# RomanArzumanyan/VALI

Hardware: AMD Instinct MI355X
Metric: nv12_to_rgb_2160p_frames_per_s (higher is better)
Workload: dtype u8; 1 GPU; BatchedFramePipeline / PySurfaceConverter.RunBatch NV12->RGB 3840x2160, BT.709 limited range, 512 frames/GPU per step (BASELINE configs[4] geometry); frames_per_gpu=512, global_batch=512, bytes_per_frame=37324800, parallelism=frame-sharded x1, RCCL broadcast of coefficients

## Files before the change

### vali_amd/csrc/common.hpp

```cpp
#pragma once
#include <hip/hip_runtime.h>
#include <stdint.h>
#include <stdio.h>
#include <string>

#include "../../include/vali_hip.h"

namespace vali {

std::string& last_error();

int fail(int code, const char* fmt, ...) __attribute__((format(printf, 2, 3)));

class DeviceScope {
public:
  explicit DeviceScope(int device);
  ~DeviceScope();
  bool ok() const { return m_ok; }

private:
  int m_prev = -1;
  bool m_switched = false;
  bool m_ok = true;
};

int stream_device(hipStream_t stream);

unsigned residency_lds_bytes(int block_threads, int waves_per_cu, unsigned min_bytes);

inline int streaming_waves_per_cu(int groups, int block, int full_lane_waves) {
  const int lanes = ((groups + block - 1) / block) * block;
  const int util_pct = groups * 100 / lanes;
  return util_pct >= 90 ? full_lane_waves : util_pct >= 70 ? full_lane_waves * 3 / 2 : full_lane_waves * 7 / 4;
}

int tuning(int key);

class TraceRange {
public:
  explicit TraceRange(const char* name);
  ~TraceRange();

private:
  bool m_pushed = false;
};

inline hipStream_t as_stream(vali_stream_t s) { return (hipStream_t)s; }

inline bool aligned16(const void* p) { return (((uintptr_t)p) & 15u) == 0; }

inline bool planes_fit_32bit(const vali_surface& s) {
  for (int c = 0; c < 3; ++c)
    if (s.plane[c] && (s.pitch[c] < 0 || (uint64_t)s.pitch[c] * (uint64_t)s.height * 3u >= (1ull << 32)))
      return false;
  return true;
}

inline bool subsampled_sizes_ok(int format, int width, int height) {
  switch (format) {
  case VALI_FMT_NV12: case VALI_FMT_P10: case VALI_FMT_P12: case VALI_FMT_YUV420: case VALI_FMT_YUV420_10BIT:
    return ((width | height) & 1) == 0;
  case VALI_FMT_YUV422:
    return (width & 1) == 0;
  default:
    return true;
  }
}

}

#define VALI_ENTRY_NAMED(stream, name)                                                       \
  ::vali::TraceRange _trace(name);                                                            \
  const int _dev = ::vali::stream_device(stream);                                             \
  if (_dev < 0)                                                                               \
    return ::vali::fail(VALI_ERR_NO_DEVICE, "%s: no usable HIP device", name);                \
  ::vali::DeviceScope scope(_dev);                                                            \
  if (!scope.ok())                                                                            \
    return ::vali::fail(VALI_ERR_NO_DEVICE, "%s: cannot select device %d", name, _dev)
#define VALI_ENTRY(stream) VALI_ENTRY_NAMED(stream, __func__)

#define VALI_HIP_CHECK(expr)                                                   \
  do {                                                                         \
    hipError_t _e = (expr);                                                    \
    if (_e != hipSuccess)                                                      \
      return ::vali::fail(VALI_ERR_RUNTIME, "%s failed: %s (%s:%d)", #expr,    \
                          hipGetErrorString(_e), __FILE__, __LINE__);          \
  } while (0)

#define VALI_REQUIRE(cond, msg)                                                \
  do {                                                                         \
    if (!(cond))                                                               \
      return ::vali::fail(VALI_ERR_INVALID_ARG, "%s: %s", __func__, msg);      \
  } while (0)

#define VALI_LAUNCH_CHECK()                                                    \
  do {                                                                         \
    hipError_t _e = hipGetLastError();                                         \
    if (_e != hipSuccess)                                                      \
      return ::vali::fail(VALI_ERR_RUNTIME, "%s: kernel launch failed: %s",    \
                          __func__, hipGetErrorString(_e));                    \
  } while (0)
```

### vali_amd/csrc/cvt_nv12_rgb.hip

```cpp
#include "common.hpp"
#include "dev_util.hpp"

namespace vali {

enum : int { LAYOUT_RGB = 0, LAYOUT_BGR = 1, LAYOUT_PLANAR = 2 };

struct Nv12RgbArgs {
  const vali_surface* d_src;
  const vali_surface* d_dst;
  vali_surface src;
  vali_surface dst;
  vali_csc csc;
  TileMap map;
  int rp;
};

template <int LAYOUT>
__device__ __forceinline__ void emit4(u32 y4, const ChromaTerm& c01, const ChromaTerm& c23,
                                      const vali_csc& k, u32* o3, u32& pr, u32& pg,
                                      u32& pb) {
  const float y0 = luma_term(ubyte_f32<0>(y4), k), y1 = luma_term(ubyte_f32<1>(y4), k),
              y2 = luma_term(ubyte_f32<2>(y4), k), y3 = luma_term(ubyte_f32<3>(y4), k);
  const float r0 = y0 + c01.rv, g0 = y0 + c01.guv, b0 = y0 + c01.bu;
  const float r1 = y1 + c01.rv, g1 = y1 + c01.guv, b1 = y1 + c01.bu;
  const float r2 = y2 + c23.rv, g2 = y2 + c23.guv, b2 = y2 + c23.bu;
  const float r3 = y3 + c23.rv, g3 = y3 + c23.guv, b3 = y3 + c23.bu;
  if constexpr (LAYOUT == LAYOUT_PLANAR) {
    u32 r = 0, g = 0, b = 0;
    r = pack_u8<0>(r0, r); r = pack_u8<1>(r1, r); r = pack_u8<2>(r2, r); r = pack_u8<3>(r3, r);
    g = pack_u8<0>(g0, g); g = pack_u8<1>(g1, g); g = pack_u8<2>(g2, g); g = pack_u8<3>(g3, g);
    b = pack_u8<0>(b0, b); b = pack_u8<1>(b1, b); b = pack_u8<2>(b2, b); b = pack_u8<3>(b3, b);
    pr = r; pg = g; pb = b;
  } else {
    const float f0 = LAYOUT == LAYOUT_RGB ? r0 : b0, l0 = LAYOUT == LAYOUT_RGB ? b0 : r0;
    const float f1 = LAYOUT == LAYOUT_RGB ? r1 : b1, l1 = LAYOUT == LAYOUT_RGB ? b1 : r1;
    const float f2 = LAYOUT == LAYOUT_RGB ? r2 : b2, l2 = LAYOUT == LAYOUT_RGB ? b2 : r2;
    const float f3 = LAYOUT == LAYOUT_RGB ? r3 : b3, l3 = LAYOUT == LAYOUT_RGB ? b3 : r3;
    u32 d0 = 0, d1 = 0, d2 = 0;
    d0 = pack_u8<0>(f0, d0); d0 = pack_u8<1>(g0, d0); d0 = pack_u8<2>(l0, d0); d0 = pack_u8<3>(f1, d0);
    d1 = pack_u8<0>(g1, d1); d1 = pack_u8<1>(l1, d1); d1 = pack_u8<2>(f2, d1); d1 = pack_u8<3>(g2, d1);
    d2 = pack_u8<0>(l2, d2); d2 = pack_u8<1>(f3, d2); d2 = pack_u8<2>(g3, d2); d2 = pack_u8<3>(l3, d2);
    o3[0] = d0; o3[1] = d1; o3[2] = d2;
  }
}

template <int LAYOUT>
__device__ __forceinline__ void convert_group(const uint4& ya, const uint4& yb, const uint4& uv, const vali_csc& k,
                                              u32 (&o0)[12], u32 (&o1)[12]) {
  const u32 yw0[4] = {ya.x, ya.y, ya.z, ya.w};
  const u32 yw1[4] = {yb.x, yb.y, yb.z, yb.w};
  const u32 uvw[4] = {uv.x, uv.y, uv.z, uv.w};
#pragma unroll
  for (int j = 0; j < 4; ++j) {
    const ChromaTerm c01 = chroma_term(ubyte_f32<0>(uvw[j]), ubyte_f32<1>(uvw[j]), k);
    const ChromaTerm c23 = chroma_term(ubyte_f32<2>(uvw[j]), ubyte_f32<3>(uvw[j]), k);
    if constexpr (LAYOUT == LAYOUT_PLANAR) {
      emit4<LAYOUT>(yw0[j], c01, c23, k, nullptr, o0[j], o0[4 + j], o0[8 + j]);
      emit4<LAYOUT>(yw1[j], c01, c23, k, nullptr, o1[j], o1[4 + j], o1[8 + j]);
    } else {
      u32 dummy;
      emit4<LAYOUT>(yw0[j], c01, c23, k, &o0[3 * j], dummy, dummy, dummy);
      emit4<LAYOUT>(yw1[j], c01, c23, k, &o1[3 * j], dummy, dummy, dummy);
    }
  }
}

template <int LAYOUT>
__global__ void __launch_bounds__(kBlock) k_nv12_rgb8(const Nv12RgbArgs a) {
  extern __shared__ uint4 dyn_lds[];
  PackedStrip* const strips = reinterpret_cast<PackedStrip*>(dyn_lds);

  u32 tile_x, tile_y, frame;
  if (!tile_of_block(a.map, tile_x, tile_y, frame))
    return;

  const uint8_t* py;
  const uint8_t* puv;
  uint8_t* pd0;
  uint8_t* pd1;
  uint8_t* pd2;
  int sp_y, sp_uv, dp, W, H;
  if (a.d_src) {
    const vali_surface* s = a.d_src + frame;
    const vali_surface* d = a.d_dst + frame;
    py = (const uint8_t*)s->plane[0]; puv = (const uint8_t*)s->plane[1];
    sp_y = s->pitch[0]; sp_uv = s->pitch[1]; W = s->width; H = s->height;
    pd0 = (uint8_t*)d->plane[0]; pd1 = (uint8_t*)d->plane[1]; pd2 = (uint8_t*)d->plane[2];
    dp = d->pitch[0];
  } else {
    py = (const uint8_t*)a.src.plane[0]; puv = (const uint8_t*)a.src.plane[1];
    sp_y = a.src.pitch[0]; sp_uv = a.src.pitch[1]; W = a.src.width; H = a.src.height;
    pd0 = (uint8_t*)a.dst.plane[0]; pd1 = (uint8_t*)a.dst.plane[1]; pd2 = (uint8_t*)a.dst.plane[2];
    dp = a.dst.pitch[0];
  }
  const vali_csc k = a.csc;

  const int lane = threadIdx.x & (kWave - 1);
  const int wave_all = threadIdx.x / kWave;
  const int wpr = (int)(blockDim.x / kWave) / a.rp;
  const int wave = wave_all;
  const int wave_g0 = (tile_x * wpr + wave_all % wpr) * kWave;
  const int groups = (W + kLanePx - 1) / kLanePx;
  if (wave_g0 >= groups)
    return;
  const int g = wave_g0 + lane;
  const int x0 = g * kLanePx;
  const int crow = tile_y * a.rp + wave_all / wpr;
  if (crow * 2 >= H)
    return;
  const int row0 = crow * 2;

  uintptr_t align_bits = (uintptr_t)py | (uintptr_t)puv | (uintptr_t)sp_y |
                         (uintptr_t)sp_uv | (uintptr_t)pd0 | (uintptr_t)dp;
  if constexpr (LAYOUT == LAYOUT_PLANAR)
    align_bits |= (uintptr_t)pd1 | (uintptr_t)pd2;
  const bool fast = ((W & (kLanePx - 1)) == 0) && ((align_bits & 15u) == 0);

  if (fast) {
    const bool lane_valid = g < groups;
    u32 o0[12], o1[12];
    if (lane_valid) {
      const uint4 ya = load16(py + (size_t)row0 * sp_y + x0);
      const uint4 yb = load16(py + (size_t)(row0 + 1) * sp_y + x0);
      const uint4 uv = load16(puv + (size_t)crow * sp_uv + x0);
      convert_group<LAYOUT>(ya, yb, uv, k, o0, o1);
    }
    if constexpr (LAYOUT == LAYOUT_PLANAR) {
      if (lane_valid) {
        uint8_t* const planes[3] = {pd0, pd1, pd2};
#pragma unroll
        for (int c = 0; c < 3; ++c) {
          uint8_t* p = planes[c] + (size_t)row0 * dp + x0;
          store16_nt(p, make_uint4(o0[4 * c], o0[4 * c + 1], o0[4 * c + 2], o0[4 * c + 3]));
          store16_nt(p + dp, make_uint4(o1[4 * c], o1[4 * c + 1], o1[4 * c + 2], o1[4 * c + 3]));
        }
      }
    } else {
      PackedStrip& strip = strips[wave];
      const int valid_lanes = min(kWave, groups - wave_g0);
      const int valid_bytes = valid_lanes * 48;
      uint8_t* rb = pd0 + (size_t)row0 * dp + (size_t)wave_g0 * 48;
      strip_store_row(strip, lane, o0, lane_valid, rb, valid_bytes);
      strip_store_row(strip, lane, o1, lane_valid, rb + dp, valid_bytes);
    }
    return;
  }

  {
    const bool lane_valid = g < groups;
    const bool cut = lane_valid && x0 + kLanePx > W;
    const int xs = cut ? max(W - kLanePx, 0) : x0;
    const int n_px = min(kLanePx, W);
    u32 o0[12], o1[12];
    if (lane_valid) {
      const uint4 ya = load16_n(py + (size_t)row0 * sp_y + xs, n_px);
      const uint4 yb = load16_n(py + (size_t)(row0 + 1) * sp_y + xs, n_px);
      const uint4 uv = load16_n(puv + (size_t)crow * sp_uv + xs, n_px);
      convert_group<LAYOUT>(ya, yb, uv, k, o0, o1);
    }
    if constexpr (LAYOUT == LAYOUT_PLANAR) {
      if (lane_valid) {
        uint8_t* const planes[3] = {pd0, pd1, pd2};
#pragma unroll
        for (int c = 0; c < 3; ++c) {
          uint8_t* p = planes[c] + (size_t)row0 * dp + xs;
          store16_n(p, make_uint4(o0[4 * c], o0[4 * c + 1], o0[4 * c + 2], o0[4 * c + 3]), n_px);
          store16_n(p + dp, make_uint4(o1[4 * c], o1[4 * c + 1], o1[4 * c + 2], o1[4 * c + 3]), n_px);
        }
      }
    } else {
      PackedStrip& strip = strips[wave];
      const int full_lanes = min(kWave, W / kLanePx - wave_g0);
      uint8_t* rb = pd0 + (size_t)row0 * dp + (size_t)wave_g0 * 48;
      strip_store_row_u(strip, lane, o0, lane_valid && !cut, rb, full_lanes * 48);
      strip_store_row_u(strip, lane, o1, lane_valid && !cut, rb + dp, full_lanes * 48);
      if (cut) {
        packed_group_store(pd0 + (size_t)row0 * dp + (size_t)xs * 3, n_px, o0);
        packed_group_store(pd0 + (size_t)(row0 + 1) * dp + (size_t)xs * 3, n_px, o1);
      }
    }
  }
}

static int launch_nv12_rgb(Nv12RgbArgs& a, int width, int height, int n, int dst_format,
                           hipStream_t stream) {
  const int groups = (width + kLanePx - 1) / kLanePx;
  int block = ((groups + kWave - 1) / kWave) * kWave;
  if (block > kBlock)
    block = kBlock;
  const int rp_env = tuning(VALI_TUNE_NV12_ROWPAIRS);
  const int row_block = block;
  a.rp = rp_env > 0 ? rp_env : kBlock / row_block;
  if (a.rp < 1 || row_block * a.rp > kBlock)
    a.rp = 1;
  a.map = make_tile_map((groups + row_block - 1) / row_block, ((height + 1) / 2 + a.rp - 1) / a.rp, (u32)n);
  block = row_block * a.rp;
  const dim3 grid = tile_grid(a.map);
  const int waves_override = tuning(VALI_TUNE_WAVES_PER_CU);
  const int waves_per_cu = waves_override > 0 ? waves_override : streaming_waves_per_cu(groups, row_block, 16);
  const unsigned lds =
      residency_lds_bytes(block, waves_per_cu, (unsigned)sizeof(PackedStrip) * (unsigned)((block + kWave - 1) / kWave));
  switch (dst_format) {
  case VALI_FMT_RGB:
    hipLaunchKernelGGL((k_nv12_rgb8<LAYOUT_RGB>), grid, dim3(block), lds, stream, a);
    break;
  case VALI_FMT_BGR:
    hipLaunchKernelGGL((k_nv12_rgb8<LAYOUT_BGR>), grid, dim3(block), lds, stream, a);
    break;
  case VALI_FMT_RGB_PLANAR:
    hipLaunchKernelGGL((k_nv12_rgb8<LAYOUT_PLANAR>), grid, dim3(block), lds, stream, a);
    break;
  default:
    return fail(VALI_ERR_UNSUPPORTED, "nv12_to_rgb: unsupported dst format %d", dst_format);
  }
  VALI_LAUNCH_CHECK();
  return VALI_OK;
}

}

using namespace vali;

extern "C" {

int vali_nv12_to_rgb(const vali_surface* src, const vali_surface* dst, const vali_csc* csc,
                     vali_stream_t stream) {
  VALI_REQUIRE(src && dst && csc, "null argument");
  VALI_REQUIRE(src->format == VALI_FMT_NV12, "src must be NV12");
  VALI_REQUIRE(src->width > 0 && src->height > 0, "empty src");
  VALI_REQUIRE(src->width == dst->width && src->height == dst->height, "src/dst size mismatch");
  VALI_REQUIRE(((src->width | src->height) & 1) == 0, "4:2:0 surfaces need even width and height");
  VALI_REQUIRE(src->plane[0] && src->plane[1] && dst->plane[0], "null plane");
  if (dst->format == VALI_FMT_RGB_PLANAR)
    VALI_REQUIRE(dst->plane[1] && dst->plane[2], "null planar plane");
  Nv12RgbArgs a = {};
  a.src = *src;
  a.dst = *dst;
  a.csc = *csc;
  hipStream_t s = as_stream(stream);
  VALI_ENTRY(s);
  return launch_nv12_rgb(a, src->width, src->height, 1, dst->format, s);
}

int vali_nv12_to_rgb_batch(const vali_surface* d_src, const vali_surface* d_dst, int n, int width,
                           int height, int dst_format, const vali_csc* csc,
                           vali_stream_t stream) {
  VALI_REQUIRE(d_src && d_dst && csc, "null argument");
  VALI_REQUIRE(width > 0 && height > 0, "empty geometry");
  VALI_REQUIRE(((width | height) & 1) == 0, "4:2:0 surfaces need even width and height");
  VALI_REQUIRE(n >= 0 && n <= 65535, "batch size out of range (0..65535)");
  if (n == 0)
    return VALI_OK;
  Nv12RgbArgs a = {};
  a.d_src = d_src;
  a.d_dst = d_dst;
  a.csc = *csc;
  hipStream_t s = as_stream(stream);
  VALI_ENTRY(s);
  return launch_nv12_rgb(a, width, height, n, dst_format, s);
}


__global__ void k_debug_quantize(const float* in, uint8_t* out, int n) {
  const int i = blockIdx.x * blockDim.x + threadIdx.x;
  if (i < n)
    out[i] = (uint8_t)quantize_u8(in[i]);
}

__global__ void k_debug_quantize_portable(const float* in, uint8_t* out, int n) {
  const int i = blockIdx.x * blockDim.x + threadIdx.x;
  if (i < n)
    out[i] = (uint8_t)quantize_u8_portable(in[i]);
}

int vali_debug_quantize_u8(const float* d_in, uint8_t* d_out, int n, vali_stream_t stream) {
  VALI_REQUIRE(d_in && d_out && n >= 0, "bad argument");
  if (!n)
    return VALI_OK;
  hipStream_t s = as_stream(stream);
  VALI_ENTRY(s);
  hipLaunchKernelGGL(k_debug_quantize, dim3((n + 255) / 256), dim3(256), 0, s, d_in, d_out, n);
  VALI_LAUNCH_CHECK();
  return VALI_OK;
}

int vali_debug_quantize_u8_portable(const float* d_in, uint8_t* d_out, int n,
                                    vali_stream_t stream) {
  VALI_REQUIRE(d_in && d_out && n >= 0, "bad argument");
  if (!n)
    return VALI_OK;
  hipStream_t s = as_stream(stream);
  VALI_ENTRY(s);
  hipLaunchKernelGGL(k_debug_quantize_portable, dim3((n + 255) / 256), dim3(256), 0, s, d_in,
                     d_out, n);
  VALI_LAUNCH_CHECK();
  return VALI_OK;
}

}
```

### vali_amd/csrc/dev_util.hpp

```cpp
#pragma once
#include <hip/hip_runtime.h>
#include <stdint.h>

#include <type_traits>

#include "../../include/vali_hip.h"

namespace vali {

typedef uint32_t u32;

constexpr int kLanePx = 16;
constexpr int kWave = 64;
constexpr int kBlock = 256;
constexpr int kWavesPerBlock = kBlock / kWave;

template <int I> __device__ __forceinline__ float ubyte_f32(u32 w) {
  return (float)((w >> (8 * I)) & 0xffu);
}

template <int I> __device__ __forceinline__ u32 ubyte(u32 w) {
  return (w >> (8 * I)) & 0xffu;
}

__device__ __forceinline__ u32 quantize_u8_portable(float v) {
  float r = __builtin_rintf(v);
  r = __builtin_fminf(__builtin_fmaxf(r, 0.0f), 255.0f);
  return (u32)r;
}

template <int SEL> __device__ __forceinline__ u32 pack_u8(float v, u32 old) {
  return __builtin_amdgcn_cvt_pk_u8_f32(v, SEL, old);
}

__device__ __forceinline__ u32 quantize_u8(float v) { return __builtin_amdgcn_cvt_pk_u8_f32(v, 0, 0u); }

struct ChromaTerm {
  float rv, guv, bu;
};

__device__ __forceinline__ ChromaTerm chroma_term(float u, float v, const vali_csc& k) {
  const float uc = u - 128.0f, vc = v - 128.0f;
  ChromaTerm t;
  t.rv = k.crv * vc;
  t.guv = __builtin_fmaf(k.cgu, uc, k.cgv * vc);
  t.bu = k.cbu * uc;
  return t;
}

__device__ __forceinline__ float luma_term(float y, const vali_csc& k) {
  return k.cy * (y - k.y0);
}

struct Lerp {
  int i0, i1;
  float a;
};

__device__ __forceinline__ Lerp make_lerp(int x, float scale, int size) {
  const float f = (float)x * scale;
  const float fl = __builtin_floorf(f);
  Lerp l;
  l.a = f - fl;
  const int i = (int)fl;
  l.i0 = min(i, size - 1);
  l.i1 = min(i + 1, size - 1);
  return l;
}

#define VALI_GLOBAL __attribute__((address_space(1)))
typedef unsigned v4u32 __attribute__((ext_vector_type(4)));
typedef unsigned v2u32 __attribute__((ext_vector_type(2)));
typedef float v4f32 __attribute__((ext_vector_type(4)));

template <typename T> __device__ __forceinline__ T gload(const void* p) {
  return *(const VALI_GLOBAL T*)p;
}
template <typename T> __device__ __forceinline__ void gstore(void* p, T v) {
  *(VALI_GLOBAL T*)p = v;
}
template <typename T> __device__ __forceinline__ T gload_u(const void* p) {
  typedef T TU __attribute__((aligned(1)));
  return *(const VALI_GLOBAL TU*)p;
}
template <typename T> __device__ __forceinline__ void gstore_u(void* p, T v) {
  typedef T TU __attribute__((aligned(1)));
  *(VALI_GLOBAL TU*)p = v;
}
template <typename T> __device__ __forceinline__ void gstore_nt(void* p, T v) {
  __builtin_nontemporal_store(v, (VALI_GLOBAL T*)p);
}
template <typename T> __device__ __forceinline__ void gstore_u_nt(void* p, T v) {
  typedef T TU __attribute__((aligned(1)));
  __builtin_nontemporal_store(v, (VALI_GLOBAL TU*)p);
}

__device__ __forceinline__ void store16_nt(void* p, uint4 v) {
  const v4u32 w = {v.x, v.y, v.z, v.w};
  __builtin_nontemporal_store(w, (v4u32*)p);
}
__device__ __forceinline__ void store16(void* p, uint4 v) { *(uint4*)p = v; }
__device__ __forceinline__ uint4 load16(const void* p) { return *(const uint4*)p; }
typedef v4u32 v4u32_u __attribute__((aligned(1)));
typedef unsigned short u16_u __attribute__((aligned(1)));
__device__ __forceinline__ uint4 load16_u(const void* p) {
  const v4u32 w = *(const v4u32_u*)p;
  return make_uint4(w.x, w.y, w.z, w.w);
}
__device__ __forceinline__ void store16_u(void* p, uint4 v) {
  const v4u32 w = {v.x, v.y, v.z, v.w};
  *(v4u32_u*)p = w;
}
__device__ __forceinline__ uint4 load_bytes16(const uint8_t* p, int n) {
  u32 w[4] = {0u, 0u, 0u, 0u};
#pragma unroll
  for (int k = 0; k < 16; ++k)
    if (k < n)
      w[k / 4] |= (u32)p[k] << (8 * (k % 4));
  return make_uint4(w[0], w[1], w[2], w[3]);
}
__device__ __forceinline__ void store_bytes16(uint8_t* p, uint4 v, int n) {
  const u32 w[4] = {v.x, v.y, v.z, v.w};
#pragma unroll
  for (int k = 0; k < 16; ++k)
    if (k < n)
      p[k] = (uint8_t)(w[k / 4] >> (8 * (k % 4)));
}
__device__ __forceinline__ uint4 load16_n(const uint8_t* p, int n) { return n >= 16 ? load16_u(p) : load_bytes16(p, n); }
__device__ __forceinline__ void store16_n(uint8_t* p, uint4 v, int n) {
  if (n >= 16) store16_u(p, v);
  else store_bytes16(p, v, n);
}
__device__ __forceinline__ uint4 gload16(const void* p) {
  const v4u32 w = *(const VALI_GLOBAL v4u32*)p;
  return make_uint4(w.x, w.y, w.z, w.w);
}
__device__ __forceinline__ uint4 gload16_nt(const void* p) {
  const v4u32 w = __builtin_nontemporal_load((const VALI_GLOBAL v4u32*)p);
  return make_uint4(w.x, w.y, w.z, w.w);
}
__device__ __forceinline__ void gstore16_nt(void* p, uint4 v) {
  const v4u32 w = {v.x, v.y, v.z, v.w};
  __builtin_nontemporal_store(w, (VALI_GLOBAL v4u32*)p);
}
__device__ __forceinline__ uint2 load8(const void* p) {
  const v2u32 w = *(const VALI_GLOBAL v2u32*)p;
  return make_uint2(w.x, w.y);
}
__device__ __forceinline__ void store8_nt(void* p, uint2 v) {
  const v2u32 w = {v.x, v.y};
  __builtin_nontemporal_store(w, (VALI_GLOBAL v2u32*)p);
}
__device__ __forceinline__ void store16f(void* p, float4 v) {
  const v4f32 w = {v.x, v.y, v.z, v.w};
  *(VALI_GLOBAL v4f32*)p = w;
}
__device__ __forceinline__ void store16f_nt(void* p, float4 v) {
  const v4f32 w = {v.x, v.y, v.z, v.w};
  __builtin_nontemporal_store(w, (VALI_GLOBAL v4f32*)p);
}
__device__ __forceinline__ float4 load16f(const void* p) {
  const v4f32 w = *(const VALI_GLOBAL v4f32*)p;
  return make_float4(w.x, w.y, w.z, w.w);
}

struct TileMap {
  u32 total;
  u32 per_xcd;
  u32 tiles_x;
  u32 per_frame;
};

__host__ __device__ inline TileMap make_tile_map(u32 tiles_x, u32 tiles_y, u32 frames = 1u) {
  TileMap m;
  m.per_frame = tiles_x * tiles_y;
  m.total = m.per_frame * frames;
  m.per_xcd = (m.total + 7u) / 8u;
  m.tiles_x = tiles_x;
  return m;
}

__host__ __device__ inline TileMap make_tile_map_linear(u32 per_frame, u32 frames) {
  TileMap m;
  m.per_frame = per_frame;
  m.total = per_frame * frames;
  m.per_xcd = (m.total + 7u) / 8u;
  m.tiles_x = 1u;
  return m;
}

inline dim3 tile_grid(const TileMap& m) { return dim3(m.per_xcd * 8u); }

__device__ __forceinline__ bool frame_tile_of_block(const TileMap& m, u32& frame, u32& tile) {
  const u32 b = blockIdx.x;
  const u32 t = (b & 7u) * m.per_xcd + (b >> 3);
  if (t >= m.total)
    return false;
  if (m.total == m.per_frame) {
    frame = 0;
    tile = t;
  } else {
    frame = t / m.per_frame;
    tile = t - frame * m.per_frame;
  }
  return true;
}

__device__ __forceinline__ bool tile_of_block(const TileMap& m, u32& tx, u32& ty, u32& frame) {
  u32 t;
  if (!frame_tile_of_block(m, frame, t))
    return false;
  if (m.tiles_x == 1u) {
    tx = 0;
    ty = t;
  } else {
    ty = t / m.tiles_x;
    tx = t - ty * m.tiles_x;
  }
  return true;
}

struct SurfRef {
  uint8_t* p[3];
  int pitch[3];
  int width, height;
};

__device__ __forceinline__ SurfRef load_surface(const vali_surface* arr, const vali_surface& one,
                                                u32 index) {
  SurfRef r;
  if (arr) {
    const vali_surface* s = arr + index;
    r.p[0] = (uint8_t*)s->plane[0]; r.p[1] = (uint8_t*)s->plane[1]; r.p[2] = (uint8_t*)s->plane[2];
    r.pitch[0] = s->pitch[0]; r.pitch[1] = s->pitch[1]; r.pitch[2] = s->pitch[2];
    r.width = s->width; r.height = s->height;
  } else {
    r.p[0] = (uint8_t*)one.plane[0]; r.p[1] = (uint8_t*)one.plane[1]; r.p[2] = (uint8_t*)one.plane[2];
    r.pitch[0] = one.pitch[0]; r.pitch[1] = one.pitch[1]; r.pitch[2] = one.pitch[2];
    r.width = one.width; r.height = one.height;
  }
  return r;
}

struct PlaneJob {
  int comp;
  int sub_x, sub_y;
  int ssub_x, ssub_y;
  int channels;
  int kind;
  u32 first_tile, tiles_x;
  float shift_x, shift_y;
  const uint8_t* sp;
  uint8_t* dp;
  int spitch, dpitch;
  const float4* xtab;
  const float4* ytab;
};

struct PlaneView {
  const uint8_t* sp;
  uint8_t* dp;
  int spitch, dpitch, sw, sh, dw, dh;
};

__device__ __forceinline__ PlaneView plane_view(const vali_surface* d_src, const vali_surface* d_dst,
                                                u32 frame, const PlaneJob& job, int sw, int sh,
                                                int dw, int dh) {
  PlaneView v;
  if (d_src) {
    const vali_surface* s = d_src + frame;
    const vali_surface* d = d_dst + frame;
    v.sp = (const uint8_t*)s->plane[job.comp];
    v.dp = (uint8_t*)d->plane[job.comp];
    v.spitch = s->pitch[job.comp];
    v.dpitch = d->pitch[job.comp];
    sw = s->width; sh = s->height; dw = d->width; dh = d->height;
  } else {
    v.sp = job.sp; v.dp = job.dp; v.spitch = job.spitch; v.dpitch = job.dpitch;
  }
  v.sw = sw >> job.ssub_x; v.sh = sh >> job.ssub_y;
  v.dw = dw >> job.sub_x; v.dh = dh >> job.sub_y;
  return v;
}

__device__ __forceinline__ bool plane_tile(const PlaneJob (&jobs)[3], int njobs, const TileMap& map,
                                           PlaneJob& job, u32& tx, u32& ty, u32& frame) {
  u32 t;
  if (!frame_tile_of_block(map, frame, t))
    return false;
  job = jobs[0];
  if (njobs > 1 && t >= jobs[1].first_tile) job = jobs[1];
  if (njobs > 2 && t >= jobs[2].first_tile) job = jobs[2];
  const u32 local = t - job.first_tile;
  ty = local / job.tiles_x;
  tx = local - ty * job.tiles_x;
  return true;
}

template <int PB> constexpr bool kStagePadded = (128 % PB) == 0;
template <bool PAD> __device__ __forceinline__ int stage_off(int a) { return PAD ? a + ((a >> 7) << 2) : a; }
constexpr int stage_alloc(int row_bytes) { return row_bytes + 4 * (row_bytes / 128); }
template <bool PAD> __device__ __forceinline__ void stage_put(uint8_t* row, int k, const uint4& q) {
  if constexpr (PAD) {
    u32* w = reinterpret_cast<u32*>(row + k * 16 + ((k >> 3) << 2));
    w[0] = q.x; w[1] = q.y; w[2] = q.z; w[3] = q.w;
  } else {
    *reinterpret_cast<uint4*>(row + k * 16) = q;
  }
}

__device__ __forceinline__ void wave_lds_sync() {
  __builtin_amdgcn_fence(__ATOMIC_RELEASE, "wavefront");
  __builtin_amdgcn_wave_barrier();
  __builtin_amdgcn_fence(__ATOMIC_ACQUIRE, "wavefront");
}

struct alignas(16) PackedStrip {
  uint4 v[kWave * 3];
};

__device__ __forceinline__ void strip_store_row(PackedStrip& strip, int lane,
                                                const u32 (&o)[12], bool lane_valid,
                                                uint8_t* row_base, int valid_bytes) {
  if (lane_valid) {
    strip.v[lane * 3 + 0] = make_uint4(o[0], o[1], o[2], o[3]);
    strip.v[lane * 3 + 1] = make_uint4(o[4], o[5], o[6], o[7]);
    strip.v[lane * 3 + 2] = make_uint4(o[8], o[9], o[10], o[11]);
  }
  wave_lds_sync();
#pragma unroll
  for (int k = 0; k < 3; ++k) {
    const int off = (k * kWave + lane) * 16;
    if (off < valid_bytes)
      store16_nt(row_base + off, strip.v[k * kWave + lane]);
  }
  wave_lds_sync();
}

__device__ __forceinline__ void strip_store_row_u(PackedStrip& strip, int lane, const u32 (&o)[12], bool lane_valid,
                                                  uint8_t* row_base, int valid_bytes) {
  if (lane_valid) {
    strip.v[lane * 3 + 0] = make_uint4(o[0], o[1], o[2], o[3]);
    strip.v[lane * 3 + 1] = make_uint4(o[4], o[5], o[6], o[7]);
    strip.v[lane * 3 + 2] = make_uint4(o[8], o[9], o[10], o[11]);
  }
  wave_lds_sync();
#pragma unroll
  for (int k = 0; k < 3; ++k) {
    const int off = (k * kWave + lane) * 16;
    if (off < valid_bytes)
      store16_u(row_base + off, strip.v[k * kWave + lane]);
  }
  wave_lds_sync();
}

__device__ __forceinline__ void strip_load_row(PackedStrip& strip, int lane,
                                               u32 (&o)[12], bool lane_valid,
                                               const uint8_t* row_base,
                                               int valid_bytes) {
#pragma unroll
  for (int k = 0; k < 3; ++k) {
    const int off = (k * kWave + lane) * 16;
    if (off < valid_bytes)
      strip.v[k * kWave + lane] = load16(row_base + off);
  }
  wave_lds_sync();
  if (lane_valid) {
    const uint4 a = strip.v[lane * 3 + 0], b = strip.v[lane * 3 + 1],
                c = strip.v[lane * 3 + 2];
    o[0] = a.x; o[1] = a.y; o[2] = a.z; o[3] = a.w;
    o[4] = b.x; o[5] = b.y; o[6] = b.z; o[7] = b.w;
    o[8] = c.x; o[9] = c.y; o[10] = c.z; o[11] = c.w;
  }
  wave_lds_sync();
}

struct StripRegs {
  uint4 v[3];
};

__device__ __forceinline__ void strip_fetch(StripRegs& r, int lane, const uint8_t* row_base,
                                            int valid_bytes) {
#pragma unroll
  for (int k = 0; k < 3; ++k) {
    const int off = (k * kWave + lane) * 16;
    r.v[k] = off < valid_bytes ? load16(row_base + off) : make_uint4(0, 0, 0, 0);
  }
}

__device__ __forceinline__ void strip_fetch_u(StripRegs& r, int lane, const uint8_t* row_base, int valid_bytes) {
#pragma unroll
  for (int k = 0; k < 3; ++k) {
    const int off = (k * kWave + lane) * 16;
    r.v[k] = off < valid_bytes ? load16_u(row_base + off) : make_uint4(0, 0, 0, 0);
  }
}

__device__ __forceinline__ void packed_group_load(const uint8_t* p, int n_px, u32 (&o)[12]) {
#pragma unroll
  for (int k = 0; k < 3; ++k) {
    const uint4 v = load16_n(p + 16 * k, n_px * 3 - 16 * k);
    o[4 * k] = v.x; o[4 * k + 1] = v.y; o[4 * k + 2] = v.z; o[4 * k + 3] = v.w;
  }
}
__device__ __forceinline__ void packed_group_store(uint8_t* p, int n_px, const u32 (&o)[12]) {
#pragma unroll
  for (int k = 0; k < 3; ++k)
    store16_n(p + 16 * k, make_uint4(o[4 * k], o[4 * k + 1], o[4 * k + 2], o[4 * k + 3]), n_px * 3 - 16 * k);
}

__device__ __forceinline__ void strip_unpack(PackedStrip& strip, int lane, const StripRegs& r,
                                             u32 (&o)[12], bool lane_valid) {
#pragma unroll
  for (int k = 0; k < 3; ++k)
    strip.v[k * kWave + lane] = r.v[k];
  wave_lds_sync();
  if (lane_valid) {
    const uint4 a = strip.v[lane * 3 + 0], b = strip.v[lane * 3 + 1], c = strip.v[lane * 3 + 2];
    o[0] = a.x; o[1] = a.y; o[2] = a.z; o[3] = a.w;
    o[4] = b.x; o[5] = b.y; o[6] = b.z; o[7] = b.w;
    o[8] = c.x; o[9] = c.y; o[10] = c.z; o[11] = c.w;
  }
  wave_lds_sync();
}

__device__ __forceinline__ void interleave3(const u32 (&a)[4], const u32 (&b)[4],
                                            const u32 (&c)[4], u32 (&o)[12]) {
#pragma unroll
  for (int j = 0; j < 4; ++j) {
    const u32 ab_lo = __builtin_amdgcn_perm(b[j], a[j], 0x05010400u);
    const u32 ab_hi = __builtin_amdgcn_perm(b[j], a[j], 0x07030602u);
    o[3 * j + 0] = __builtin_amdgcn_perm(c[j], ab_lo, 0x02040100u);
    const u32 t = __builtin_amdgcn_perm(c[j], ab_lo, 0x00000503u);
    o[3 * j + 1] = __builtin_amdgcn_perm(ab_hi, t, 0x05040100u);
    o[3 * j + 2] = __builtin_amdgcn_perm(c[j], ab_hi, 0x07030206u);
  }
}

__device__ __forceinline__ void deinterleave3(const u32 (&o)[12], u32 (&a)[4],
                                              u32 (&b)[4], u32 (&c)[4]) {
#pragma unroll
  for (int j = 0; j < 4; ++j) {
    const u32 d0 = o[3 * j], d1 = o[3 * j + 1], d2 = o[3 * j + 2];
    const u32 a01 = __builtin_amdgcn_perm(d1, d0, 0x00060300u);
    a[j] = __builtin_amdgcn_perm(d2, a01, 0x05020100u);
    const u32 b01 = __builtin_amdgcn_perm(d1, d0, 0x00070401u);
    b[j] = __builtin_amdgcn_perm(d2, b01, 0x06020100u);
    const u32 c01 = __builtin_amdgcn_perm(d1, d0, 0x00000502u);
    c[j] = __builtin_amdgcn_perm(d2, c01, 0x07040100u);
  }
}

template <typename T> __device__ __forceinline__ u32 finish_bits(float v);
template <> __device__ __forceinline__ u32 finish_bits<uint8_t>(float v) { return quantize_u8(v); }
template <> __device__ __forceinline__ u32 finish_bits<uint16_t>(float v) {
  const float r = __builtin_fminf(__builtin_fmaxf(__builtin_rintf(v), 0.0f), 65535.0f);
  return (u32)r;
}
template <> __device__ __forceinline__ u32 finish_bits<float>(float v) { return __float_as_uint(v); }

template <typename T, int C>
__device__ __forceinline__ void store_px4(uint8_t* dst, const float (&res)[4][C], u32 mask) {
  constexpr int E = (int)sizeof(T), N = 4 * C, NB = N * E, PER = 4 / E;
  u32 w[NB / 4];
#pragma unroll
  for (int k = 0; k < NB / 4; ++k)
    w[k] = 0;
#pragma unroll
  for (int k = 0; k < N; ++k) {
    const float v = res[k / C][k % C];
    if constexpr (E == 1)
      w[k / 4] = __builtin_amdgcn_cvt_pk_u8_f32(v, (u32)(k % 4), w[k / 4]);
    else
      w[k / PER] |= finish_bits<T>(v) << (8 * E * (k % PER));
  }
  constexpr u32 kAlign = NB % 16 == 0 ? 15u : (NB % 8 == 0 ? 7u : 3u);
  if (mask == 0xfu && (((uintptr_t)dst) & kAlign) == 0) {
    if constexpr (NB == 16) {
      const v4u32 q = {w[0], w[1], w[2], w[3]};
      gstore_nt<v4u32>(dst, q);
    } else if constexpr (NB % 16 == 0) {
#pragma unroll
      for (int k = 0; k < NB / 16; ++k) {
        const v4u32 q = {w[4 * k], w[4 * k + 1], w[4 * k + 2], w[4 * k + 3]};
        ((VALI_GLOBAL v4u32*)dst)[k] = q;
      }
    } else if constexpr (NB == 8) {
      const v2u32 q = {w[0], w[1]};
      gstore_nt<v2u32>(dst, q);
    } else if constexpr (NB % 8 == 0) {
#pragma unroll
      for (int k = 0; k < NB / 8; ++k) {
        const v2u32 q = {w[2 * k], w[2 * k + 1]};
        ((VALI_GLOBAL v2u32*)dst)[k] = q;
      }
    } else if constexpr (NB == 12) {
      typedef unsigned v3u32 __attribute__((ext_vector_type(3)));
      const v3u32 q = {w[0], w[1], w[2]};
      gstore_nt<v3u32>(dst, q);
    } else if constexpr (NB == 4) {
      gstore_nt<u32>(dst, w[0]);
    } else {
#pragma unroll
      for (int k = 0; k < NB / 4; ++k)
        ((VALI_GLOBAL u32*)dst)[k] = w[k];
    }
    return;
  }
#pragma unroll
  for (int k = 0; k < N; ++k)
    if (mask & (1u << (k / C))) {
      const u32 bits = w[k / PER] >> (8 * E * (k % PER));
      ((VALI_GLOBAL T*)dst)[k] = __builtin_bit_cast(T, (typename std::conditional<E == 1, uint8_t, typename std::conditional<E == 2, uint16_t, u32>::type>::type)bits);
    }
}

template <typename T, int C> struct PairLoad {
  static constexpr bool kMerged = (sizeof(T) == 1 && C <= 3) || (sizeof(T) == 2 && C == 1);
};
template <typename T, int C>
__device__ __forceinline__ void load_tap_pair(const uint8_t* row, int i, int sw, float (&t0)[C], float (&t1)[C]) {
  typedef uint16_t u16_unaligned __attribute__((aligned(1)));
  typedef u32 u32_unaligned __attribute__((aligned(1)));
  typedef unsigned long long u64_unaligned __attribute__((aligned(1)));
  const int base = min(i, sw - 2);
  const bool edge = i != base;
  if constexpr (sizeof(T) == 1 && C == 1) {
    const u32 w = *(const VALI_GLOBAL u16_unaligned*)(row + base);
    t1[0] = (float)(w >> 8);
    t0[0] = edge ? t1[0] : (float)(w & 0xffu);
  } else if constexpr (sizeof(T) == 1 && C == 2) {
    const u32 w = *(const VALI_GLOBAL u32_unaligned*)(row + 2 * base);
    t1[0] = ubyte_f32<2>(w); t1[1] = ubyte_f32<3>(w);
    t0[0] = edge ? t1[0] : ubyte_f32<0>(w);
    t0[1] = edge ? t1[1] : ubyte_f32<1>(w);
  } else if constexpr (sizeof(T) == 2 && C == 1) {
    const u32 w = *(const VALI_GLOBAL u32_unaligned*)(row + 2 * base);
    t1[0] = (float)(w >> 16);
    t0[0] = edge ? t1[0] : (float)(w & 0xffffu);
  } else {
    const int want = 3 * base, start = min(want, 3 * sw - 8);
    const unsigned long long q = *(const VALI_GLOBAL u64_unaligned*)(row + start) >> (8 * (want - start));
    const u32 lo = (u32)q, hi = (u32)(q >> 32);
    t1[0] = ubyte_f32<3>(lo); t1[1] = ubyte_f32<0>(hi); t1[2] = ubyte_f32<1>(hi);
    t0[0] = edge ? t1[0] : ubyte_f32<0>(lo);
    t0[1] = edge ? t1[1] : ubyte_f32<1>(lo);
    t0[2] = edge ? t1[2] : ubyte_f32<2>(lo);
  }
}


}
```

Before: 168,500 frames/s.

## Flatten NV12→RGB work into linear item tiles with magic-number row division

Adds a linear work mapping for aligned, non-ragged inputs. Each lane handles one 16-pixel group indexed over all (row-pair, group) items of a frame, and a host-validated multiply-high replaces the division by groups-per-row. At 3840 width, the row-tied blocks of 256 lanes carry 240 groups, so about 6% of lanes sit idle; the flat mapping is meant to keep every lane busy. In exchange, a wave's packed RGB stores can straddle row boundaries, and each lane computes per-piece destination addresses. The old row-tied path is kept for ragged or unaligned cases and for explicit row-pair tuning.

```diff
diff --git a/vali_amd/csrc/common.hpp b/vali_amd/csrc/common.hpp
--- a/vali_amd/csrc/common.hpp
+++ b/vali_amd/csrc/common.hpp
@@ -32,6 +32,30 @@
   const int lanes = ((groups + block - 1) / block) * block;
   const int util_pct = groups * 100 / lanes;
   return util_pct >= 90 ? full_lane_waves : util_pct >= 70 ? full_lane_waves * 3 / 2 : full_lane_waves * 7 / 4;
+}
+
+inline uint32_t linear_item_multiplier(uint32_t d, uint32_t n) {
+  thread_local uint32_t seen_d = 0, seen_n = 0, seen_m = 0;
+  if (d == seen_d && n == seen_n)
+    return seen_m;
+  uint32_t m = 0;
+  if (d > 1) {
+    m = (uint32_t)((1ull << 32) / d) + 1u;
+    for (uint32_t i = 0, q = 0, r = 0; i < n; ++i) {
+      if ((uint32_t)(((uint64_t)i * m) >> 32) != q) {
+        m = 0;
+        break;
+      }
+      if (++r == d) {
+        r = 0;
+        ++q;
+      }
+    }
+  }
+  seen_d = d;
+  seen_n = n;
+  seen_m = m;
+  return m;
 }
 
 int tuning(int key);
diff --git a/vali_amd/csrc/cvt_nv12_rgb.hip b/vali_amd/csrc/cvt_nv12_rgb.hip
--- a/vali_amd/csrc/cvt_nv12_rgb.hip
+++ b/vali_amd/csrc/cvt_nv12_rgb.hip
@@ -13,6 +13,18 @@
   vali_csc csc;
   TileMap map;
   int rp;
+  u32 groups, pairs;
+  u32 items;
+  u32 div_mul;
+};
+
+struct Nv12RgbFrame {
+  const uint8_t* py;
+  const uint8_t* puv;
+  uint8_t* pd0;
+  uint8_t* pd1;
+  uint8_t* pd2;
+  int sp_y, sp_uv, dp, W, H;
 };
 
 template <int LAYOUT>
@@ -66,38 +78,71 @@
 }
 
 template <int LAYOUT>
-__global__ void __launch_bounds__(kBlock) k_nv12_rgb8(const Nv12RgbArgs a) {
-  extern __shared__ uint4 dyn_lds[];
-  PackedStrip* const strips = reinterpret_cast<PackedStrip*>(dyn_lds);
-
-  u32 tile_x, tile_y, frame;
-  if (!tile_of_block(a.map, tile_x, tile_y, frame))
-    return;
-
-  const uint8_t* py;
-  const uint8_t* puv;
-  uint8_t* pd0;
-  uint8_t* pd1;
-  uint8_t* pd2;
-  int sp_y, sp_uv, dp, W, H;
-  if (a.d_src) {
-    const vali_surface* s = a.d_src + frame;
-    const vali_surface* d = a.d_dst + frame;
-    py = (const uint8_t*)s->plane[0]; puv = (const uint8_t*)s->plane[1];
-    sp_y = s->pitch[0]; sp_uv = s->pitch[1]; W = s->width; H = s->height;
-    pd0 = (uint8_t*)d->plane[0]; pd1 = (uint8_t*)d->plane[1]; pd2 = (uint8_t*)d->plane[2];
-    dp = d->pitch[0];
-  } else {
-    py = (const uint8_t*)a.src.plane[0]; puv = (const uint8_t*)a.src.plane[1];
-    sp_y = a.src.pitch[0]; sp_uv = a.src.pitch[1]; W = a.src.width; H = a.src.height;
-    pd0 = (uint8_t*)a.dst.plane[0]; pd1 = (uint8_t*)a.dst.plane[1]; pd2 = (uint8_t*)a.dst.plane[2];
-    dp = a.dst.pitch[0];
-  }
-  const vali_csc k = a.csc;
+__device__ __forceinline__ void linear_tile(const Nv12RgbFrame& f, const vali_csc& k, const Nv12RgbArgs& a, u32 tile,
+                                            bool aligned, PackedStrip* strips) {
+  const int lane = threadIdx.x & (kWave - 1);
+  const int wave = threadIdx.x / kWave;
+  const u32 i0 = tile * (u32)kBlock + (u32)(wave * kWave);
+  if (i0 >= a.items || (u32)f.W != a.groups * (u32)kLanePx || (u32)f.H != a.pairs * 2u)
+    return;
+  const u32 i = i0 + (u32)lane;
+  const bool lane_valid = i < a.items;
+  u32 crow, g;
+  item_row_group(i, a.groups, a.div_mul, crow, g);
+  const size_t x0 = (size_t)g * kLanePx;
+  const size_t row0 = (size_t)crow * 2;
+  u32 o0[12], o1[12];
+  if (lane_valid) {
+    const uint4 ya = load16_u(f.py + row0 * f.sp_y + x0);
+    const uint4 yb = load16_u(f.py + (row0 + 1) * f.sp_y + x0);
+    const uint4 uv = load16_u(f.puv + (size_t)crow * f.sp_uv + x0);
+    convert_group<LAYOUT>(ya, yb, uv, k, o0, o1);
+  }
+  if constexpr (LAYOUT == LAYOUT_PLANAR) {
+    if (lane_valid) {
+      uint8_t* const planes[3] = {f.pd0, f.pd1, f.pd2};
+#pragma unroll
+      for (int c = 0; c < 3; ++c) {
+        uint8_t* p = planes[c] + row0 * f.dp + x0;
+        const uint4 v0 = make_uint4(o0[4 * c], o0[4 * c + 1], o0[4 * c + 2], o0[4 * c + 3]);
+        const uint4 v1 = make_uint4(o1[4 * c], o1[4 * c + 1], o1[4 * c + 2], o1[4 * c + 3]);
+        if (aligned) {
+          store16_nt(p, v0);
+          store16_nt(p + f.dp, v1);
+        } else {
+          store16_u(p, v0);
+          store16_u(p + f.dp, v1);
+        }
+      }
+    }
+  } else {
+    uint8_t* piece[3];
+#pragma unroll
+    for (int kk = 0; kk < 3; ++kk) {
+      const u32 q = (u32)(kk * kWave + lane), j = q / 3u, part = q - 3u * j;
+      u32 prow, pg;
+      item_row_group(i0 + j, a.groups, a.div_mul, prow, pg);
+      piece[kk] = f.pd0 + (size_t)prow * 2 * f.dp + (size_t)pg * 48 + part * 16;
+    }
+    const int valid_bytes = (int)min((u32)kWave, a.items - i0) * 48;
+    PackedStrip& strip = strips[wave];
+    strip_store_pieces(strip, lane, o0, lane_valid, piece, 0, valid_bytes, aligned);
+    strip_store_pieces(strip, lane, o1, lane_valid, piece, (size_t)f.dp, valid_bytes, aligned);
+  }
+}
+
+template <int LAYOUT>
+__device__ __forceinline__ void row_tied_tile(const Nv12RgbFrame& f, const vali_csc& k, bool fast, int tile_x, int tile_y,
+                                              int rp, int wpr, PackedStrip* strips) {
+  const uint8_t* const py = f.py;
+  const uint8_t* const puv = f.puv;
+  uint8_t* const pd0 = f.pd0;
+  uint8_t* const pd1 = f.pd1;
+  uint8_t* const pd2 = f.pd2;
+  const int sp_y = f.sp_y, sp_uv = f.sp_uv, dp = f.dp, W = f.W, H = f.H;
 
   const int lane = threadIdx.x & (kWave - 1);
   const int wave_all = threadIdx.x / kWave;
-  const int wpr = (int)(blockDim.x / kWave) / a.rp;
   const int wave = wave_all;
   const int wave_g0 = (tile_x * wpr + wave_all % wpr) * kWave;
   const int groups = (W + kLanePx - 1) / kLanePx;
@@ -105,16 +150,10 @@
     return;
   const int g = wave_g0 + lane;
   const int x0 = g * kLanePx;
-  const int crow = tile_y * a.rp + wave_all / wpr;
+  const int crow = tile_y * rp + wave_all / wpr;
   if (crow * 2 >= H)
     return;
   const int row0 = crow * 2;
-
-  uintptr_t align_bits = (uintptr_t)py | (uintptr_t)puv | (uintptr_t)sp_y |
-                         (uintptr_t)sp_uv | (uintptr_t)pd0 | (uintptr_t)dp;
-  if constexpr (LAYOUT == LAYOUT_PLANAR)
-    align_bits |= (uintptr_t)pd1 | (uintptr_t)pd2;
-  const bool fast = ((W & (kLanePx - 1)) == 0) && ((align_bits & 15u) == 0);
 
   if (fast) {
     const bool lane_valid = g < groups;
@@ -182,22 +221,82 @@
   }
 }
 
+template <int LAYOUT>
+__global__ void __launch_bounds__(kBlock) k_nv12_rgb8(const Nv12RgbArgs a) {
+  extern __shared__ uint4 dyn_lds[];
+  PackedStrip* const strips = reinterpret_cast<PackedStrip*>(dyn_lds);
+
+  u32 frame, tile;
+  if (!frame_tile_of_block(a.map, frame, tile))
+    return;
+
+  Nv12RgbFrame f;
+  if (a.d_src) {
+    const vali_surface* s = a.d_src + frame;
+    const vali_surface* d = a.d_dst + frame;
+    f.py = (const uint8_t*)s->plane[0]; f.puv = (const uint8_t*)s->plane[1];
+    f.sp_y = s->pitch[0]; f.sp_uv = s->pitch[1]; f.W = s->width; f.H = s->height;
+    f.pd0 = (uint8_t*)d->plane[0]; f.pd1 = (uint8_t*)d->plane[1]; f.pd2 = (uint8_t*)d->plane[2];
+    f.dp = d->pitch[0];
+  } else {
+    f.py = (const uint8_t*)a.src.plane[0]; f.puv = (const uint8_t*)a.src.plane[1];
+    f.sp_y = a.src.pitch[0]; f.sp_uv = a.src.pitch[1]; f.W = a.src.width; f.H = a.src.height;
+    f.pd0 = (uint8_t*)a.dst.plane[0]; f.pd1 = (uint8_t*)a.dst.plane[1]; f.pd2 = (uint8_t*)a.dst.plane[2];
+    f.dp = a.dst.pitch[0];
+  }
+  const vali_csc k = a.csc;
+
+  uintptr_t align_bits = (uintptr_t)f.py | (uintptr_t)f.puv | (uintptr_t)f.sp_y |
+                         (uintptr_t)f.sp_uv | (uintptr_t)f.pd0 | (uintptr_t)f.dp;
+  if constexpr (LAYOUT == LAYOUT_PLANAR)
+    align_bits |= (uintptr_t)f.pd1 | (uintptr_t)f.pd2;
+  const bool fast = ((f.W & (kLanePx - 1)) == 0) && ((align_bits & 15u) == 0);
+
+  if (a.rp == 0) {
+    linear_tile<LAYOUT>(f, k, a, tile, fast, strips);
+  } else {
+    const u32 tile_y = a.map.tiles_x == 1u ? tile : tile / a.map.tiles_x;
+    row_tied_tile<LAYOUT>(f, k, fast, (int)(tile - tile_y * a.map.tiles_x), (int)tile_y, a.rp,
+                          (int)(blockDim.x / kWave) / a.rp, strips);
+  }
+}
+
 static int launch_nv12_rgb(Nv12RgbArgs& a, int width, int height, int n, int dst_format,
                            hipStream_t stream) {
   const int groups = (width + kLanePx - 1) / kLanePx;
-  int block = ((groups + kWave - 1) / kWave) * kWave;
-  if (block > kBlock)
+  const int rp_env = tuning(VALI_TUNE_NV12_ROWPAIRS);
+  const int waves_override = tuning(VALI_TUNE_WAVES_PER_CU);
+  const uint64_t items = (uint64_t)groups * (uint64_t)(height / 2);
+  bool ragged = (width & (kLanePx - 1)) != 0;
+  if (!a.d_src) {
+    uintptr_t align_bits = (uintptr_t)a.src.plane[0] | (uintptr_t)a.src.plane[1] | (uintptr_t)a.src.pitch[0] |
+                           (uintptr_t)a.src.pitch[1] | (uintptr_t)a.dst.plane[0] | (uintptr_t)a.dst.pitch[0];
+    if (dst_format == VALI_FMT_RGB_PLANAR)
+      align_bits |= (uintptr_t)a.dst.plane[1] | (uintptr_t)a.dst.plane[2];
+    ragged = ragged || (align_bits & 15u) != 0;
+  }
+  int block, waves_per_cu;
+  if (rp_env <= 0 && !ragged && items < (1ull << 31)) {
+    a.rp = 0;
+    a.groups = (u32)groups;
+    a.pairs = (u32)(height / 2);
+    a.items = (u32)items;
+    a.div_mul = linear_item_multiplier(a.groups, a.items);
+    a.map = make_tile_map_linear((a.items + (u32)kBlock - 1u) / (u32)kBlock, (u32)n);
     block = kBlock;
-  const int rp_env = tuning(VALI_TUNE_NV12_ROWPAIRS);
-  const int row_block = block;
-  a.rp = rp_env > 0 ? rp_env : kBlock / row_block;
-  if (a.rp < 1 || row_block * a.rp > kBlock)
-    a.rp = 1;
-  a.map = make_tile_map((groups + row_block - 1) / row_block, ((height + 1) / 2 + a.rp - 1) / a.rp, (u32)n);
-  block = row_block * a.rp;
+    waves_per_cu = waves_override > 0 ? waves_override : 16;
+  } else {
+    int row_block = ((groups + kWave - 1) / kWave) * kWave;
+    if (row_block > kBlock)
+      row_block = kBlock;
+    a.rp = rp_env > 0 ? rp_env : kBlock / row_block;
+    if (a.rp < 1 || row_block * a.rp > kBlock)
+      a.rp = 1;
+    a.map = make_tile_map((groups + row_block - 1) / row_block, ((height + 1) / 2 + a.rp - 1) / a.rp, (u32)n);
+    block = row_block * a.rp;
+    waves_per_cu = waves_override > 0 ? waves_override : streaming_waves_per_cu(groups, row_block, 16);
+  }
   const dim3 grid = tile_grid(a.map);
-  const int waves_override = tuning(VALI_TUNE_WAVES_PER_CU);
-  const int waves_per_cu = waves_override > 0 ? waves_override : streaming_waves_per_cu(groups, row_block, 16);
   const unsigned lds =
       residency_lds_bytes(block, waves_per_cu, (unsigned)sizeof(PackedStrip) * (unsigned)((block + kWave - 1) / kWave));
   switch (dst_format) {
diff --git a/vali_amd/csrc/dev_util.hpp b/vali_amd/csrc/dev_util.hpp
--- a/vali_amd/csrc/dev_util.hpp
+++ b/vali_amd/csrc/dev_util.hpp
@@ -335,6 +335,32 @@
       store16_nt(row_base + off, strip.v[k * kWave + lane]);
   }
   wave_lds_sync();
+}
+
+__device__ __forceinline__ void strip_store_pieces(PackedStrip& strip, int lane, const u32 (&o)[12], bool lane_valid,
+                                                   uint8_t* const (&piece)[3], size_t row_off, int valid_bytes, bool aligned) {
+  if (lane_valid) {
+    strip.v[lane * 3 + 0] = make_uint4(o[0], o[1], o[2], o[3]);
+    strip.v[lane * 3 + 1] = make_uint4(o[4], o[5], o[6], o[7]);
+    strip.v[lane * 3 + 2] = make_uint4(o[8], o[9], o[10], o[11]);
+  }
+  wave_lds_sync();
+#pragma unroll
+  for (int k = 0; k < 3; ++k) {
+    const int off = (k * kWave + lane) * 16;
+    if (off < valid_bytes) {
+      if (aligned)
+        store16_nt(piece[k] + row_off, strip.v[k * kWave + lane]);
+      else
+        store16_u(piece[k] + row_off, strip.v[k * kWave + lane]);
+    }
+  }
+  wave_lds_sync();
+}
+
+__device__ __forceinline__ void item_row_group(u32 i, u32 groups, u32 mul, u32& row, u32& group) {
+  row = mul ? __umulhi(i, mul) : i / groups;
+  group = i - row * groups;
 }
 
 __device__ __forceinline__ void strip_store_row_u(PackedStrip& strip, int lane, const u32 (&o)[12], bool lane_valid,
```

New measurement: 169,200 frames/s (median of 2 runs). About the same (+0.4%).
